# aerius-labs/indexed-merkle-tree-halo2

Hardware: AMD Instinct MI355X
Metric: indexed-tree insertions/sec at depth=32 (bn256::Fr) (higher is better)
Workload: dtype u32 limbs (9 x 29-bit, Montgomery mod p), 64-bit accumulate

## Files before the change

indexed-merkle-tree-halo2_amd/csrc/imt_device.hpp:

```cpp
#pragma once
#include <cstddef>
#include <cstdint>
#include "imt_consts.hpp"

#if defined(__HIPCC__)
#include <hip/hip_runtime.h>
#define IMT_HD __host__ __device__ __forceinline__
#else
#define IMT_HD inline
#endif

namespace imt {
namespace dev {

#define IMT_P29_0 0x10000001u
#define IMT_P29_1 0x1f0fac9fu
#define IMT_P29_2 0x0e5c2450u
#define IMT_P29_3 0x07d090f3u
#define IMT_P29_4 0x1585d283u
#define IMT_P29_5 0x02db40c0u
#define IMT_P29_6 0x00a6e141u
#define IMT_P29_7 0x0e5c2634u
#define IMT_P29_8 0x0030644eu
constexpr uint32_t N0INV29 = 0x0fffffffu;
constexpr uint32_t N0INV32 = 0xefffffffu;

IMT_HD constexpr uint32_t p29(int i) {
    return i == 0 ? IMT_P29_0 : i == 1 ? IMT_P29_1 : i == 2 ? IMT_P29_2 : i == 3 ? IMT_P29_3 :
           i == 4 ? IMT_P29_4 : i == 5 ? IMT_P29_5 : i == 6 ? IMT_P29_6 : i == 7 ? IMT_P29_7 : IMT_P29_8;
}


template <bool WIDE_M>
IMT_HD uint32_t mont_digit(uint64_t acc) {
    return WIDE_M ? (uint32_t)acc * N0INV32 : (((uint32_t)acc * N0INV29) & MASK29);
}

}
}
#if defined(__HIP_DEVICE_COMPILE__) && !defined(IMT_NO_MONT_ASM)
#define IMT_MONT_ASM 1
#include "imt_mont_asm.hpp"
#include "imt_mont_asm_rec.hpp"
#endif
namespace imt {
namespace dev {

template <int NT, bool ADD, bool WIDE_M = true>
IMT_HD void mont_dot(Fe& r, const Fe* a, const Fe* b, const Fe& addend) {
    uint32_t m[NL];
    uint64_t acc = 0;
#pragma unroll
    for (int k = 0; k < NL; k++) {
#pragma unroll
        for (int t = 0; t < NT; t++) {
#pragma unroll
            for (int i = 0; i <= k; i++) acc += (uint64_t)a[t].v[i] * b[t].v[k - i];
        }
#pragma unroll
        for (int i = 0; i < k; i++) acc += (uint64_t)m[i] * p29(k - i);
        m[k] = mont_digit<WIDE_M>(acc);
        acc += (uint64_t)m[k] * p29(0);
        acc >>= 29;
    }
#pragma unroll
    for (int k = NL; k < 2 * NL - 1; k++) {
#pragma unroll
        for (int t = 0; t < NT; t++) {
#pragma unroll
            for (int i = k - (NL - 1); i < NL; i++) acc += (uint64_t)a[t].v[i] * b[t].v[k - i];
        }
#pragma unroll
        for (int i = k - (NL - 1); i < NL; i++) acc += (uint64_t)m[i] * p29(k - i);
        if (ADD) acc += addend.v[k - NL];
        r.v[k - NL] = (uint32_t)acc & MASK29;
        acc >>= 29;
    }
    if (ADD) acc += addend.v[NL - 1];
    r.v[NL - 1] = (uint32_t)acc;
}

IMT_HD void mont_mul(Fe& r, const Fe& a, const Fe& b) {
#ifdef IMT_MONT_ASM
    masm::mul_vv(r, &a, &b);
#else
    mont_dot<1, false>(r, &a, &b, a);
#endif
}

template <int NT, bool ADD, bool WIDE_M = true>
IMT_HD void mont_dot_uc(Fe& r, const Fe* c, const Fe* v, const Fe& addend) {
#ifdef IMT_MONT_ASM
    static_assert((NT == 3 && !ADD && WIDE_M) || (NT == 4 && WIDE_M) || (NT == 2 && ADD && !WIDE_M),
                  "no assembly form for this shape");
    if constexpr (NT == 3) masm::dot3_uc(r, c, v);
    else if constexpr (NT == 4 && ADD) masm::dot4_add_uc(r, c, v, addend);
    else if constexpr (NT == 4) masm::dot4_uc(r, c, v);
    else masm::dot2_add_uc_narrow(r, c, v, addend);
#else
    mont_dot<NT, ADD, WIDE_M>(r, c, v, addend);
#endif
}

IMT_HD void mont_sqr(Fe& r, const Fe& a) {
#ifdef IMT_MONT_ASM
    masm::sqr_v(r, a);
    return;
#endif
    uint32_t m[NL], a2[NL];
#pragma unroll
    for (int i = 0; i < NL; i++) a2[i] = a.v[i] << 1;
    uint64_t acc = 0;
#pragma unroll
    for (int k = 0; k < NL; k++) {
#pragma unroll
        for (int i = 0; 2 * i < k; i++) acc += (uint64_t)a2[i] * a.v[k - i];
        if ((k & 1) == 0) acc += (uint64_t)a.v[k / 2] * a.v[k / 2];
#pragma unroll
        for (int i = 0; i < k; i++) acc += (uint64_t)m[i] * p29(k - i);
        m[k] = mont_digit<true>(acc);
        acc += (uint64_t)m[k] * p29(0);
        acc >>= 29;
    }
#pragma unroll
    for (int k = NL; k < 2 * NL - 1; k++) {
#pragma unroll
        for (int i = k - (NL - 1); 2 * i < k; i++) acc += (uint64_t)a2[i] * a.v[k - i];
        if ((k & 1) == 0) acc += (uint64_t)a.v[k / 2] * a.v[k / 2];
#pragma unroll
        for (int i = k - (NL - 1); i < NL; i++) acc += (uint64_t)m[i] * p29(k - i);
        r.v[k - NL] = (uint32_t)acc & MASK29;
        acc >>= 29;
    }
    r.v[NL - 1] = (uint32_t)acc;
}

IMT_HD void mont_redc(Fe& r, const Fe& a) {
    uint32_t m[NL];
    uint64_t acc = 0;
#pragma unroll
    for (int k = 0; k < NL; k++) {
        acc += a.v[k];
#pragma unroll
        for (int i = 0; i < k; i++) acc += (uint64_t)m[i] * p29(k - i);
        m[k] = mont_digit<false>(acc);
        acc += (uint64_t)m[k] * p29(0);
        acc >>= 29;
    }
#pragma unroll
    for (int k = NL; k < 2 * NL - 1; k++) {
#pragma unroll
        for (int i = k - (NL - 1); i < NL; i++) acc += (uint64_t)m[i] * p29(k - i);
        r.v[k - NL] = (uint32_t)acc & MASK29;
        acc >>= 29;
    }
    r.v[NL - 1] = (uint32_t)acc;
}

IMT_HD void add_lazy(Fe& r, const Fe& a, const Fe& b) {
#pragma unroll
    for (int i = 0; i < NL; i++) r.v[i] = a.v[i] + b.v[i];
}

IMT_HD void normalize(Fe& a) {
#pragma unroll
    for (int i = 0; i < NL - 1; i++) {
        a.v[i + 1] += a.v[i] >> 29;
        a.v[i] &= MASK29;
    }
}

IMT_HD bool geq_p(const Fe& a) {
    bool ge = true;
#pragma unroll
    for (int i = 0; i < NL; i++) {
        uint32_t pi = p29(i);
        if (a.v[i] != pi) ge = a.v[i] > pi;
    }
    return ge;
}

IMT_HD void sub_p(Fe& a) {
    uint32_t borrow = 0;
#pragma unroll
    for (int i = 0; i < NL; i++) {
        uint32_t d = a.v[i] - p29(i) - borrow;
        borrow = (i < NL - 1) ? (d >> 31) : 0;
        a.v[i] = (i < NL - 1) ? (d & MASK29) : d;
    }
}

template <int SH>
IMT_HD constexpr uint32_t p29_shl(int i) {
    return i == 0 ? ((p29(0) << SH) & MASK29)
         : i < NL - 1 ? (((p29(i) << SH) | (p29(i - 1) >> (29 - SH))) & MASK29)
                      : ((p29(i) << SH) | (p29(i - 1) >> (29 - SH)));
}
template <int SH>
IMT_HD void cond_sub_p_shl(Fe& a) {
    bool ge = true;
#pragma unroll
    for (int i = 0; i < NL; i++) {
        const uint32_t pi = p29_shl<SH>(i);
        if (a.v[i] != pi) ge = a.v[i] > pi;
    }
    if (ge) {
        uint32_t borrow = 0;
#pragma unroll
        for (int i = 0; i < NL; i++) {
            uint32_t d = a.v[i] - p29_shl<SH>(i) - borrow;
            borrow = (i < NL - 1) ? (d >> 31) : 0;
            a.v[i] = (i < NL - 1) ? (d & MASK29) : d;
        }
    }
}

IMT_HD void canonicalize(Fe& a) {
    cond_sub_p_shl<4>(a);
    cond_sub_p_shl<3>(a);
    cond_sub_p_shl<2>(a);
    cond_sub_p_shl<1>(a);
    cond_sub_p_shl<0>(a);
}

IMT_HD void unpack(Fe& r, const uint32_t w[8]) {
#pragma unroll
    for (int i = 0; i < NL; i++) {
        const int bit = 29 * i, wi = bit >> 5, sh = bit & 31;
        uint32_t lo = w[wi] >> sh;
        if (sh > 3 && wi + 1 < 8) lo |= w[wi + 1] << (32 - sh);
        r.v[i] = lo & MASK29;
    }
}
IMT_HD void pack(uint32_t w[8], const Fe& a) {
#pragma unroll
    for (int j = 0; j < 8; j++) {
        const int lo_limb = (32 * j) / 29, off = 32 * j - 29 * lo_limb;
        uint32_t x = a.v[lo_limb] >> off;
        const int have = 29 - off;
        if (have < 32 && lo_limb + 1 < NL) x |= a.v[lo_limb + 1] << have;
        if (have + 29 < 32 && lo_limb + 2 < NL) x |= a.v[lo_limb + 2] << (have + 29);
        w[j] = x;
    }
}

struct alignas(16) Word4 { uint32_t x, y, z, w; };
IMT_HD void load_packed(Fe& r, const void* ptr) {
    const Word4* q = reinterpret_cast<const Word4*>(ptr);
    Word4 x = q[0], y = q[1];
    uint32_t w[8] = {x.x, x.y, x.z, x.w, y.x, y.y, y.z, y.w};
    unpack(r, w);
}
IMT_HD void store_packed(void* ptr, const Fe& a) {
    uint32_t w[8];
    pack(w, a);
    Word4* q = reinterpret_cast<Word4*>(ptr);
    q[0] = Word4{w[0], w[1], w[2], w[3]};
    q[1] = Word4{w[4], w[5], w[6], w[7]};
}



IMT_HD void sbox(Fe& x) {
    Fe x2, x4;
    mont_sqr(x2, x);
    mont_sqr(x4, x2);
    mont_mul(x, x4, x);
}

IMT_HD constexpr uint32_t pc29(int i) { return i == 0 ? (1u << 29) - p29(0) : MASK29 - p29(i); }
constexpr uint32_t FOLD_RECIP = 1354;

IMT_HD void fold_p(Fe& a) {
    const uint32_t q = (uint32_t)(((uint64_t)a.v[NL - 1] * FOLD_RECIP) >> 32);
    uint64_t acc = 0;
#pragma unroll
    for (int i = 0; i < NL; i++) {
        acc = (acc >> 29) + a.v[i] + (uint64_t)q * pc29(i);
        a.v[i] = i < NL - 1 ? (uint32_t)acc & MASK29 : (uint32_t)(acc - ((uint64_t)q << 29));
    }
}

IMT_HD void permute(const PoseidonConsts& pc, Fe s[3], const Fe* first_rc) {
    constexpr int NSTEP = RF + RP;
    Fe z3;
#pragma unroll
    for (int i = 0; i < NL; i++) z3.v[i] = 0;
#pragma unroll 1
    for (int st = 0; st < NSTEP; st++) {
        if (st < RF / 2 || st >= RF / 2 + RP) {
            const int fr = st < RF / 2 ? st : st - RP;
            if (fr == RF / 2) {
                const Fe v[3] = {s[0], s[1], z3};
                const Fe zl = s[2];
#pragma unroll 1
                for (int i = 0; i < 2; i++) {
                    Fe n;
                    mont_dot_uc<3, false>(n, pc.rec_exit[i], v, v[0]);
                    add_lazy(n, n, zl);
                    normalize(n);
                    s[1] = s[2]; s[2] = n;
                }
            }
            const Fe* rc = (st == 0) ? first_rc : pc.sc_rc[fr];
            add_lazy(s[0], s[0], rc[0]);
            add_lazy(s[1], s[1], rc[1]);
            add_lazy(s[2], s[2], rc[2]);
            sbox(s[0]); sbox(s[1]); sbox(s[2]);
            const Fe(*mat)[3] = pc.sc_mats[fr];
            Fe n0, n1, n2;
            if (fr == 0 || fr == RF / 2) {
                mont_dot_uc<3, false>(n0, mat[0], s, s[0]);
            } else {
                add_lazy(n0, s[0], s[1]);
                add_lazy(n0, n0, s[2]);
                normalize(n0);
            }
            mont_dot_uc<3, false>(n1, mat[1], s, s[0]);
            mont_dot_uc<3, false>(n2, mat[2], s, s[0]);
            s[0] = n0; s[1] = n1; s[2] = n2;
        } else {
            const int r = st - RF / 2;
            Fe z, w;
            add_lazy(z, s[0], pc.rec_k[r]);
            sbox(z);
            if (r >= 2) {
                const Fe v[4] = {s[0], s[1], z3, s[2]};
                mont_dot_uc<4, true>(w, pc.rec_c[r], v, z);
            } else if (r == 1) {
                const Fe v[2] = {s[0], s[2]};
                Fe e;
                add_lazy(e, z3, z);
                mont_dot_uc<2, true, false>(w, pc.rec_c[1], v, e);
            } else {
                add_lazy(w, s[1], z);
                normalize(w);
            }
            s[1] = s[0]; s[0] = w; z3 = s[2]; s[2] = z;
        }
    }
}

IMT_HD void hash23(const PoseidonConsts& pc, Fe& out, const Fe& a, const Fe& b, const Fe& c, bool three) {
    Fe s[3] = {pc.cap0, a, b};
#pragma unroll 1
    for (int blk = 0; blk < 2; blk++) {
        const Fe* rc0 = pc.rc_full[0];
        if (blk == 1) {
            if (three) {
                add_lazy(s[1], s[1], c);
                add_lazy(s[2], s[2], pc.one);
                normalize(s[1]);
                normalize(s[2]);
            } else {
                rc0 = pc.rc_h2p2;
            }
        }
        permute(pc, s, rc0);
    }
    out = s[1];
    canonicalize(out);
}
IMT_HD void hash23_stashed(const PoseidonConsts& pc, Fe& out, const Fe& a, const Fe& b, bool three,
                           const uint32_t* stash, unsigned stride) {
    Fe s[3] = {pc.cap0, a, b};
#pragma unroll 1
    for (int blk = 0; blk < 2; blk++) {
        const Fe* rc0 = pc.rc_full[0];
        if (blk == 1) {
            if (three) {
                Fe c;
#pragma unroll
                for (int i = 0; i < NL; i++) c.v[i] = stash[(size_t)i * stride];
                add_lazy(s[1], s[1], c);
                add_lazy(s[2], s[2], pc.one);
                normalize(s[1]);
                normalize(s[2]);
            } else {
                rc0 = pc.rc_h2p2;
            }
        }
        permute(pc, s, rc0);
    }
    out = s[1];
    canonicalize(out);
}
IMT_HD void hash2(const PoseidonConsts& pc, Fe& out, const Fe& a, const Fe& b) { hash23(pc, out, a, b, a, false); }
IMT_HD void hash3(const PoseidonConsts& pc, Fe& out, const Fe& a, const Fe& b, const Fe& c) { hash23(pc, out, a, b, c, true); }

enum : unsigned { FMT_CANONICAL = 0, FMT_MONT256 = 1, FMT_DEVICE = 2 };

IMT_HD bool load_fe(const PoseidonConsts& pc, Fe& r, const void* ptr, unsigned fmt) {
    Fe raw;
    load_packed(raw, ptr);
    bool ok = !geq_p(raw) && (raw.v[NL - 1] >> 24) == 0;
    if (fmt == FMT_DEVICE) { r = raw; return ok; }
    mont_mul(r, raw, fmt == FMT_CANONICAL ? pc.from_canon : pc.from_mont256);
    canonicalize(r);
    return ok;
}
IMT_HD void store_fe(const PoseidonConsts& pc, void* ptr, const Fe& a, unsigned fmt) {
    if (fmt == FMT_DEVICE) { store_packed(ptr, a); return; }
    Fe t;
    mont_mul(t, a, fmt == FMT_CANONICAL ? pc.int_one : pc.to_mont256);
    canonicalize(t);
    store_packed(ptr, t);
}

IMT_HD bool fe_eq(const Fe& a, const Fe& b) {
    uint32_t d = 0;
#pragma unroll
    for (int i = 0; i < NL; i++) d |= a.v[i] ^ b.v[i];
    return d == 0;
}
IMT_HD bool fe_is_zero(const Fe& a) {
    uint32_t d = 0;
#pragma unroll
    for (int i = 0; i < NL; i++) d |= a.v[i];
    return d == 0;
}

}
}
```

indexed-merkle-tree-halo2_amd/csrc/imt_kernels.hip:

```cpp
#include <algorithm>
#include <hip/hip_runtime.h>
#include <hip/hip_ext.h>

#include "imt_device.hpp"
#include "imt_trace_device.hpp"
#include "imt_launch.hpp"
#include "imt_sweep.hpp"
#if defined(__HIP_DEVICE_COMPILE__)
#include "imt_coop_device.hpp"
#endif

namespace imt {

__constant__ dev::PoseidonConsts g_pc;
__constant__ dev::TraceConsts g_tc;

namespace {
using namespace dev;

#ifndef IMT_BLOCK
#define IMT_BLOCK 256
#endif
#ifndef IMT_HASH_WAVES
#define IMT_HASH_WAVES __attribute__((amdgpu_waves_per_eu(5, 5)))
// ... 417 lines not shown
        Fe rt;
        ok &= load_fe(g_pc, rt, root + i * (size_t)root_stride, fmt_in);
        if (!fe_eq(cur, rt)) fail |= 0x02;
        fail_out[i] = (uint8_t)fail;
        if (root_out) store_fe(g_pc, root_out + i * 32, cur, fmt_out);
    }
    flag_err(err, ok);
#endif
}

__global__ void __launch_bounds__(BLOCK) k_split128(const uint8_t* __restrict__ vals, uint8_t* __restrict__ q,
                                                    uint8_t* __restrict__ r, size_t n, unsigned fmt, int* err) {
    const size_t i = gtid();
    if (i >= n) return;
    Fe x, xi;
    bool ok = load_fe(g_pc, x, vals + i * 32, fmt);
    to_int(xi, x);
    uint32_t w[8];
    pack(w, xi);
    Fe lo, hi, t;
    const uint32_t wl[8] = {w[0], w[1], w[2], w[3], 0, 0, 0, 0};
    const uint32_t wh[8] = {w[4], w[5], w[6], w[7], 0, 0, 0, 0};
    unpack(t, wl);
    mont_mul(lo, t, g_pc.from_canon);
    canonicalize(lo);
    unpack(t, wh);
    mont_mul(hi, t, g_pc.from_canon);
    canonicalize(hi);
    store_fe(g_pc, r + i * 32, lo, fmt);
    store_fe(g_pc, q + i * 32, hi, fmt);
    flag_err(err, ok);
}

__global__ IMT_HASH_WAVES void __launch_bounds__(BLOCK)
k_insert_chains(const uint8_t* __restrict__ low_leaf, const uint64_t* __restrict__ low_index,
                const uint8_t* __restrict__ low_sib, const uint8_t* __restrict__ new_leaf,
                const uint64_t* __restrict__ new_index, const uint64_t* __restrict__ new_path_index,
                const uint8_t* __restrict__ new_sib, launch::SibLayout lay, unsigned depth, size_t n,
                uint8_t* __restrict__ trace, unsigned fmt_in, int* err) {
    const size_t i = gtid();
    if (i >= n) return;
    const int chain = blockIdx.y;
    __shared__ uint32_t stash[NL][BLOCK];
    bool ok = true;
    Fe cur;
    const uint8_t* sib = chain < 2 ? low_sib : new_sib;
    const uint64_t* index = chain < 2 ? low_index : new_path_index;
    const int leaf_row = chain == 0 ? 0 : chain == 1 ? 2 : 5, root_row = chain == 0 ? 1 : chain == 1 ? 3 : chain == 2 ? 4 : 6;
    if (chain == 2) cur = g_pc.zero_leaf;
    auto load_leaf = [=](Fe& a, Fe& b, Fe& c, bool& okk) {
        const size_t it = gtid_again();
        const uint8_t* const p0 = (chain == 3 ? new_leaf : low_leaf) + it * 96;
        okk &= load_fe(g_pc, a, p0, fmt_in);
        if (chain == 1) {
            okk &= load_fe(g_pc, b, new_leaf + it * 96, fmt_in);
            fe_from_u64(c, new_index[it]);
        } else {
            okk &= load_fe(g_pc, b, p0 + 32, fmt_in);
            okk &= load_fe(g_pc, c, p0 + 64, fmt_in);
        }
    };
    auto store_leaf = [=](const Fe& h) { store_packed(trace + ((size_t)leaf_row * n + gtid_again()) * 32, h); };
    chain_inline(cur, chain != 2, load_leaf, store_leaf, index, 0, sib, lay, depth, fmt_in, ok, &stash[0][threadIdx.x]);
    store_packed(trace + ((size_t)root_row * n + gtid_again()) * 32, cur);
    flag_err(err, ok);
}

__global__ IMT_COOP_WAVES void __launch_bounds__(BLOCK)
k_insert_chains_coop(const uint8_t* __restrict__ low_leaf, const uint64_t* __restrict__ low_index,
                     const uint8_t* __restrict__ low_sib, const uint8_t* __restrict__ new_leaf,
                     const uint64_t* __restrict__ new_index, const uint64_t* __restrict__ new_path_index,
                     const uint8_t* __restrict__ new_sib, launch::SibLayout lay, unsigned depth, size_t n,
                     uint8_t* __restrict__ trace, unsigned fmt_in, int* err) {
#if defined(__HIP_DEVICE_COMPILE__)
    __shared__ uint32_t tab[coop::TAB_DWORDS];
    coop::tab_fill(tab, g_pc);
    const size_t t = gtid();
    const size_t i = t >> 2;
    if (i >= n) return;
    const unsigned role = (unsigned)t & 3u, ri = role == 3u ? 0u : role;
    const int chain = blockIdx.y;
    bool ok = true;
    const uint8_t* sib = chain < 2 ? low_sib : new_sib;
    const uint64_t idx = chain < 2 ? low_index[i] : new_path_index[i];
    uint8_t* leaf_out = nullptr;
    uint8_t* root_out;
    Fe cur, X, C3, o;
    C3 = g_pc.one;
    if (chain == 2) {
        cur = g_pc.zero_leaf;
        root_out = trace + (4 * n + i) * 32;
    } else {
        if (chain == 1) {
            ok &= load_fe(g_pc, X, (ri == 2u ? new_leaf : low_leaf) + (i * 3 + 0) * 32, fmt_in);
            fe_from_u64(C3, new_index[i]);
            leaf_out = trace + (2 * n + i) * 32;
            root_out = trace + (3 * n + i) * 32;
        } else {
            const uint8_t* lf = chain == 0 ? low_leaf : new_leaf;
            ok &= load_fe(g_pc, X, lf + i * 96 + (ri == 2u ? 32 : 0), fmt_in);
            ok &= load_fe(g_pc, C3, lf + i * 96 + 64, fmt_in);
            if (ri == 1u) ok &= load_fe(g_pc, o, lf + i * 96 + 32, fmt_in);
            leaf_out = trace + ((chain == 0 ? 0 : 5) * n + i) * 32;
            root_out = trace + ((chain == 0 ? 1 : 6) * n + i) * 32;
        }
        coop::hash23(tab, o, X, C3, true, ri);
        coop::quad_bcast<1>(cur, o);
        if (role == 1u) store_packed(leaf_out, cur);
    }
#pragma unroll 1
    for (unsigned l = 0; l < depth; l++) {
        Fe sv;
        ok &= load_fe(g_pc, sv, sib + ((uint64_t)l * lay.level_stride + i * lay.item_stride) * 32, fmt_in);
        const bool right = (idx >> l) & 1;
        const bool take_sv = (ri == 2u) != right;
#pragma unroll
        for (int q = 0; q < NL; q++) X.v[q] = take_sv ? sv.v[q] : cur.v[q];
        coop::hash23(tab, o, X, C3, false, ri);
        coop::quad_bcast<1>(cur, o);
    }
    if (role == 1u) store_packed(root_out, cur);
    flag_err(err, ok);
#endif
}

__global__ void __launch_bounds__(BLOCK)
k_insert_check(const uint8_t* __restrict__ old_root, const uint8_t* __restrict__ low_leaf,
               const uint8_t* __restrict__ new_root, const uint8_t* __restrict__ new_leaf,
               const uint8_t* __restrict__ is_largest, size_t n, const uint8_t* __restrict__ trace,
               uint8_t* __restrict__ fail_out, unsigned fmt_in, int* err) {
    const size_t i = gtid();
    if (i >= n) return;
    bool ok = true;
    Fe low[3], nl[3], r0, r1, t;
#pragma unroll
    for (int j = 0; j < 3; j++) {
        ok &= load_fe(g_pc, low[j], low_leaf + (i * 3 + j) * 32, fmt_in);
        ok &= load_fe(g_pc, nl[j], new_leaf + (i * 3 + j) * 32, fmt_in);
    }
    ok &= load_fe(g_pc, r0, old_root + i * 32, fmt_in);
    ok &= load_fe(g_pc, r1, new_root + i * 32, fmt_in);
    unsigned fail = 0;
    Fe nvi, lvi, lni;
    to_int(nvi, nl[0]); to_int(lvi, low[0]); to_int(lni, low[1]);
    const unsigned s = is_largest[i];
    if (s > 1) fail |= 0x80;
    if (!(s ? fe_is_zero(low[1]) : int_lt(nvi, lni))) fail |= 0x01;
    if (!int_lt(lvi, nvi)) fail |= 0x04;
    load_packed(t, trace + (1 * n + i) * 32);
    if (!fe_eq(t, r0)) fail |= 0x02;
    Fe interim, z;
    load_packed(interim, trace + (3 * n + i) * 32);
    load_packed(z, trace + (4 * n + i) * 32);
    if (!fe_eq(z, interim)) fail |= 0x08;
    if (!fe_eq(nl[1], low[1])) fail |= 0x10;
    if (!fe_eq(nl[2], low[2])) fail |= 0x20;
    load_packed(t, trace + (6 * n + i) * 32);
    if (!fe_eq(t, r1)) fail |= 0x40;
    fail_out[i] = (uint8_t)fail;
    flag_err(err, ok);
}

__global__ IMT_HASH_WAVES void __launch_bounds__(BLOCK) k_tree_level(const uint8_t* __restrict__ prev, uint8_t* __restrict__ next,
                                                      size_t n_parents) {
    const size_t i = gtid();
    if (i >= n_parents) return;
    Fe a, b, o;
    load_packed(a, prev + (2 * i) * 32);
    load_packed(b, prev + (2 * i + 1) * 32);
    hash23_stashed(g_pc, o, a, b, false, nullptr, 0);
    store_packed(next + i * 32, o);
}

__device__ __forceinline__ void force_vector(Fe& x) {
#pragma unroll
    for (int i = 0; i < NL; i++) asm volatile("" : "+v"(x.v[i]));
}

__global__ IMT_HASH_WAVES void k_zero_chain(uint8_t* out, unsigned depth) {
#if defined(__HIP_DEVICE_COMPILE__)
    __shared__ uint32_t tab[coop::TAB_DWORDS];
    coop::tab_fill(tab, g_pc);
    if (blockIdx.x != 0 || threadIdx.x >= 4) return;
    const unsigned role = threadIdx.x, ri = role == 3u ? 0u : role;
    Fe cur = g_pc.zero_leaf;
    force_vector(cur);
    if (role == 1u) store_packed(out, cur);
#pragma unroll 1
    for (unsigned l = 0; l < depth; l++) {
        Fe o;
        coop::hash23(tab, o, cur, cur, false, ri);
        coop::quad_bcast<1>(cur, o);
        if (role == 1u) store_packed(out + (size_t)(l + 1) * 32, cur);
    }
#endif
}

__global__ IMT_HASH_WAVES void k_extend_root(uint8_t* cur_io, const uint8_t* zero, unsigned from, unsigned to) {
    if (threadIdx.x != 0 || blockIdx.x != 0) return;
    Fe cur;
    load_packed(cur, cur_io);
    force_vector(cur);
#pragma unroll 1
    for (unsigned l = from; l < to; l++) {
        Fe z, o;
        load_packed(z, zero + (size_t)l * 32);
        hash23_stashed(g_pc, o, cur, z, false, nullptr, 0);
        cur = o;
    }
    store_packed(cur_io, cur);
}

__global__ void __launch_bounds__(BLOCK) k_gather_proof(launch::TreeView tv, const uint64_t* __restrict__ index,
                                                        size_t n, unsigned depth, uint8_t* __restrict__ out,
                                                        launch::SibLayout lay, unsigned fmt_out) {
    const size_t t = gtid();
    if (t >= n * depth) return;
    const size_t i = t % n;
    const unsigned l = (unsigned)(t / n);
    const uint64_t s = ((index[i] - tv.index_base) >> l) ^ 1;
    const uint8_t* src = s < tv.len[l] ? tv.nodes + (tv.off[l] + s) * 32 : tv.zero + (size_t)l * 32;
    Fe x;
    load_packed(x, src);
    store_fe(g_pc, out + ((uint64_t)l * lay.level_stride + i * lay.item_stride) * 32, x, fmt_out);
}

__global__ void k_write_helpers(uint64_t index, unsigned depth, uint8_t* out, unsigned fmt_out) {
    const unsigned l = threadIdx.x + blockIdx.x * blockDim.x;
    if (l >= depth) return;
    Fe x;
    fe_from_u64(x, ((index >> l) & 1) ? 0 : 1);
    store_fe(g_pc, out + (size_t)l * 32, x, fmt_out);
}


__global__ void __launch_bounds__(BLOCK) k_fill_level(uint8_t* __restrict__ nodes, size_t n,
                                                      const uint8_t* __restrict__ zero_l) {
    const size_t i = gtid();
    if (i >= n) return;
    const Word4* z = reinterpret_cast<const Word4*>(zero_l);
    Word4* o = reinterpret_cast<Word4*>(nodes + i * 32);
    o[0] = z[0];
    o[1] = z[1];
}

__global__ void __launch_bounds__(BLOCK) k_merge_level(sweep::LevelTable in, sweep::LevelOut out, uint32_t total) {
    const size_t k = gtid();
    if (k >= total) return;
    sweep::merge_element(in, out, (uint32_t)k, total);
}

__global__ void __launch_bounds__(BLOCK)
k_writeback(const uint8_t* __restrict__ val_l, const uint32_t* __restrict__ from,
            const uint32_t* __restrict__ node_below, uint8_t* __restrict__ tree_l, uint32_t total) {
    const size_t kp = gtid();
    if (kp >= total) return;
    const uint32_t f = from[kp];
    if (!(f & sweep::LAST_BIT)) return;
    const Word4* s = reinterpret_cast<const Word4*>(val_l + (size_t)(f & ~sweep::LAST_BIT) * 32);
    Word4* d = reinterpret_cast<Word4*>(tree_l + (size_t)node_below[kp] * 32);
    d[0] = s[0];
    d[1] = s[1];
}

__global__ IMT_HASH_WAVES void __launch_bounds__(BLOCK) k_sweep(launch::SweepArgs a) {
    __shared__ uint32_t stash[NL][BLOCK];
    const size_t t = gtid();
    if (t >= a.count) return;
    const uint32_t x = a.begin + (uint32_t)t;
    Fe A, B, o;
    if (a.mode == launch::SWEEP_LEAVES) {
        const uint8_t* p = a.pre + (size_t)a.time0[x] * 96;
        Fe C;
        bool ok = load_fe(g_pc, A, p, a.fmt_in);
        ok &= load_fe(g_pc, B, p + 32, a.fmt_in);
        ok &= load_fe(g_pc, C, p + 64, a.fmt_in);
#pragma unroll
        for (int i = 0; i < NL; i++) stash[i][threadIdx.x] = C.v[i];
        flag_err(a.err, ok);
    } else {
        uint32_t k = x, n = 0, e = x;
        const uint8_t* sp = a.zero_l;
        if (a.from) {
            k = a.from[x] & ~sweep::LAST_BIT;
            n = a.node_below[x];
            e = a.time_next[x];
            const int32_t ss = a.sibsrc[x];
            const uint64_t sn = (uint64_t)(n ^ 1u);
            sp = ss >= 0 ? a.val_in + (size_t)ss * 32 : (sn < a.len_l ? a.tree_l + sn * 32 : a.zero_l);
        }
        Fe cur, sv;
        load_packed(cur, a.val_in + (size_t)k * 32);
        load_packed(sv, sp);
        if (x == a.last_event && a.node_in) store_packed(a.node_in, cur);
        const bool right = n & 1u;
#pragma unroll
        for (int i = 0; i < NL; i++) {
            A.v[i] = right ? sv.v[i] : cur.v[i];
            B.v[i] = right ? cur.v[i] : sv.v[i];
        }
        uint8_t* row = (e & 1u) ? a.new_sib : a.low_sib;
        if (row) store_fe(g_pc, row + ((uint64_t)a.level * a.lay.level_stride + (uint64_t)(e >> 1) * a.lay.item_stride) * 32, sv, a.fmt_out);
    }
    hash23_stashed(g_pc, o, A, B, a.mode == launch::SWEEP_LEAVES, &stash[0][threadIdx.x], BLOCK);
    store_packed(a.val_out + (size_t)x * 32, o);
    if (x == a.last_event && a.node_out) store_packed(a.node_out, o);
}

__global__ IMT_HASH_WAVES void __launch_bounds__(BLOCK) k_sweep_coop(launch::SweepArgs a) {
#if defined(__HIP_DEVICE_COMPILE__)
    __shared__ uint32_t tab[coop::TAB_DWORDS];
    coop::tab_fill(tab, g_pc);
    const size_t t = gtid();
    const size_t q = t >> 2;
    if (q >= a.count) return;
    const unsigned role = (unsigned)t & 3u, ri = role == 3u ? 0u : role;
    const uint32_t x = a.begin + (uint32_t)q;
    Fe X, C3, o;
    C3 = g_pc.one;
    if (a.mode == launch::SWEEP_LEAVES) {
        const uint8_t* p = a.pre + (size_t)a.time0[x] * 96;
        bool ok = load_fe(g_pc, X, p + (ri == 2u ? 32 : 0), a.fmt_in);
        ok &= load_fe(g_pc, C3, p + 64, a.fmt_in);
        if (ri == 1u) ok &= load_fe(g_pc, o, p + 32, a.fmt_in);
        flag_err(a.err, ok);
    } else {
        uint32_t k = x, n = 0, e = x;
        const uint8_t* sp = a.zero_l;
        if (a.from) {
            k = a.from[x] & ~sweep::LAST_BIT;
            n = a.node_below[x];
            e = a.time_next[x];
            const int32_t ss = a.sibsrc[x];
            const uint64_t sn = (uint64_t)(n ^ 1u);
            sp = ss >= 0 ? a.val_in + (size_t)ss * 32 : (sn < a.len_l ? a.tree_l + sn * 32 : a.zero_l);
        }
        Fe cur, sv;
        load_packed(cur, a.val_in + (size_t)k * 32);
        load_packed(sv, sp);
        const bool right = n & 1u;
        const bool take_sv = (ri == 2u) != right;
#pragma unroll
        for (int i = 0; i < NL; i++) X.v[i] = take_sv ? sv.v[i] : cur.v[i];
        if (role == 0u) {
            if (x == a.last_event && a.node_in) store_packed(a.node_in, cur);
            uint8_t* row = (e & 1u) ? a.new_sib : a.low_sib;
            if (row) store_fe(g_pc, row + ((uint64_t)a.level * a.lay.level_stride + (uint64_t)(e >> 1) * a.lay.item_stride) * 32, sv, a.fmt_out);
        }
    }
    coop::hash23(tab, o, X, C3, a.mode == launch::SWEEP_LEAVES, ri);
    if (role == 1u) {
        store_packed(a.val_out + (size_t)x * 32, o);
        if (x == a.last_event && a.node_out) store_packed(a.node_out, o);
    }
#endif
}

__global__ void __launch_bounds__(BLOCK)
k_emit_roots(const uint8_t* __restrict__ val, uint32_t e_begin, uint32_t e_count, uint32_t total,
             uint8_t* __restrict__ old_root, uint8_t* __restrict__ interim_root, uint8_t* __restrict__ new_root,
             unsigned fmt_out, uint8_t* __restrict__ roots_dev, uint8_t* __restrict__ node_store) {
    const size_t t = gtid();
    if (t >= e_count) return;
    const uint32_t e = e_begin + (uint32_t)t;
    Fe cur;
    load_packed(cur, val + (size_t)e * 32);
    if (e == total - 1 && node_store) store_packed(node_store, cur);
    if (roots_dev) { store_packed(roots_dev + (size_t)e * 32, cur); return; }
    const uint32_t i = e >> 1;
    if (e & 1u) {
        if (new_root) store_fe(g_pc, new_root + (size_t)i * 32, cur, fmt_out);
        if (old_root && (size_t)i + 1 < (size_t)(total >> 1)) store_fe(g_pc, old_root + ((size_t)i + 1) * 32, cur, fmt_out);
    } else {
        if (interim_root) store_fe(g_pc, interim_root + (size_t)i * 32, cur, fmt_out);
    }
}

__global__ IMT_HASH_WAVES void __launch_bounds__(BLOCK) k_apply_level(launch::ApplyArgs a) {
    __shared__ uint32_t stash[NL][BLOCK];
    const size_t j = gtid();
    if (j >= a.bound || j >= *a.count) return;
    const uint64_t p = a.list[j];
    if (p >= a.len_out) return;
    Fe A, B, o;
    if (a.mode == launch::APPLY_LEAVES) {
        const uint8_t* q = a.pre + (size_t)a.src[j] * 96;
        Fe C;
        bool ok = load_fe(g_pc, A, q, a.fmt_in);
        ok &= load_fe(g_pc, B, q + 32, a.fmt_in);
        ok &= load_fe(g_pc, C, q + 64, a.fmt_in);
#pragma unroll
        for (int i = 0; i < NL; i++) stash[i][threadIdx.x] = C.v[i];
        flag_err(a.err, ok);
    } else {
        const uint64_t c0 = 2 * p, c1 = 2 * p + 1;
        load_packed(A, c0 < a.len_in ? a.tree_in + c0 * 32 : a.zero_in);
        load_packed(B, c1 < a.len_in ? a.tree_in + c1 * 32 : a.zero_in);
    }
    hash23_stashed(g_pc, o, A, B, a.mode == launch::APPLY_LEAVES, &stash[0][threadIdx.x], BLOCK);
    store_packed(a.tree_out + p * 32, o);
}

__global__ IMT_HASH_WAVES void __launch_bounds__(BLOCK) k_apply_level_coop(launch::ApplyArgs a) {
#if defined(__HIP_DEVICE_COMPILE__)
    __shared__ uint32_t tab[coop::TAB_DWORDS];
    coop::tab_fill(tab, g_pc);
    const size_t t = gtid();
    const size_t j = t >> 2;
    if (j >= a.bound || j >= *a.count) return;
    const unsigned role = (unsigned)t & 3u, ri = role == 3u ? 0u : role;
    const uint64_t p = a.list[j];
    if (p >= a.len_out) return;
    Fe X, C3, o;
    C3 = g_pc.one;
    if (a.mode == launch::APPLY_LEAVES) {
        const uint8_t* q = a.pre + (size_t)a.src[j] * 96;
        bool ok = load_fe(g_pc, X, q + (ri == 2u ? 32 : 0), a.fmt_in);
        ok &= load_fe(g_pc, C3, q + 64, a.fmt_in);
        if (ri == 1u) ok &= load_fe(g_pc, o, q + 32, a.fmt_in);
        flag_err(a.err, ok);
    } else {
        const uint64_t ch = 2 * p + (ri == 2u ? 1u : 0u);
        load_packed(X, ch < a.len_in ? a.tree_in + ch * 32 : a.zero_in);
    }
    coop::hash23(tab, o, X, C3, a.mode == launch::APPLY_LEAVES, ri);
    if (role == 1u) store_packed(a.tree_out + p * 32, o);
#endif
}

__global__ IMT_HASH_WAVES void k_apply_top(uint8_t* nodes, const uint64_t* __restrict__ off, const uint64_t* __restrict__ len,
                                           const uint8_t* __restrict__ zero, unsigned from, unsigned to) {
#if defined(__HIP_DEVICE_COMPILE__)
    __shared__ uint32_t tab[coop::TAB_DWORDS];
    coop::tab_fill(tab, g_pc);
    if (blockIdx.x != 0 || threadIdx.x >= 4) return;
    const unsigned role = threadIdx.x, ri = role == 3u ? 0u : role;
    Fe cur;
    load_packed(cur, nodes + off[from] * 32);
#pragma unroll 1
    for (unsigned l = from; l < to; l++) {
        Fe z, X, o;
        load_packed(z, l == from && len[l] > 1 ? nodes + (off[l] + 1) * 32 : zero + (size_t)l * 32);
        coop::sel(X, ri == 2u, z, cur);
        coop::hash23(tab, o, X, X, false, ri);
        coop::quad_bcast<1>(cur, o);
        if (role == 1u) store_packed(nodes + off[l + 1] * 32, cur);
    }
#endif
}

__global__ IMT_HASH_WAVES void __launch_bounds__(BLOCK)
k_lift_roots(uint8_t* __restrict__ old_root, uint8_t* __restrict__ interim_root, uint8_t* __restrict__ new_root,
             uint32_t n, const uint8_t* __restrict__ top, uint64_t pos_bits, unsigned levels, unsigned fmt, int* err) {
    const size_t t = gtid();
    const uint32_t n_int = interim_root ? n : 0, n_new = new_root ? n : 0;
    const uint32_t n_old = old_root ? (new_root ? 1u : n) : 0;
    if (t >= (size_t)n_int + n_new + n_old) return;
    uint8_t* row;
    uint8_t* also = nullptr;
    if (t < n_int) {
        row = interim_root + t * 32;
    } else if (t < (size_t)n_int + n_new) {
        const size_t i = t - n_int;
        row = new_root + i * 32;
        if (old_root && i + 1 < n) also = old_root + (i + 1) * 32;
    } else {
        row = old_root + (t - n_int - n_new) * 32;
    }
    Fe cur;
    bool ok = load_fe(g_pc, cur, row, fmt);
#pragma unroll 1
    for (unsigned j = 0; j < levels; j++) {
        Fe sv, a, b, o;
        load_packed(sv, top + (size_t)j * 32);
        const bool right = (pos_bits >> j) & 1;
#pragma unroll
        for (int i = 0; i < NL; i++) {
            a.v[i] = right ? sv.v[i] : cur.v[i];
            b.v[i] = right ? cur.v[i] : sv.v[i];
        }
        hash23_stashed(g_pc, o, a, b, false, nullptr, 0);
        cur = o;
    }
    store_fe(g_pc, row, cur, fmt);
    if (also) store_fe(g_pc, also, cur, fmt);
    flag_err(err, ok);
}

__global__ void __launch_bounds__(BLOCK)
k_fill_sib_rows(uint8_t* __restrict__ sib, launch::SibLayout lay, unsigned first_level, unsigned levels, uint32_t n,
                const uint8_t* __restrict__ top, unsigned fmt_out) {
    const size_t t = gtid();
    if (t >= (size_t)n * levels) return;
    const uint32_t i = (uint32_t)(t % n);
    const unsigned j = (unsigned)(t / n);
    Fe x;
    load_packed(x, top + (size_t)j * 32);
    store_fe(g_pc, sib + ((uint64_t)(first_level + j) * lay.level_stride + (uint64_t)i * lay.item_stride) * 32, x, fmt_out);
}

__global__ void k_mix_roots(const uint8_t* __restrict__ before, const uint8_t* __restrict__ after,
                            uint8_t* __restrict__ mixed, uint32_t n_sub, uint32_t self, unsigned fmt_in, int* err) {
    const uint32_t r = blockIdx.x * blockDim.x + threadIdx.x;
    if (r >= n_sub) return;
    Fe x;
    const bool ok = load_fe(g_pc, x, (r < self ? after : before) + (size_t)r * 32, fmt_in);
    store_packed(mixed + (size_t)r * 32, x);
    flag_err(err, ok);
}

__global__ void k_pick_top(const uint8_t* __restrict__ levels_buf, uint32_t n_sub, uint32_t self, unsigned k,
                           unsigned levels, const uint8_t* __restrict__ zero, unsigned sub_depth,
                           uint8_t* __restrict__ top) {
    const unsigned j = threadIdx.x;
    if (j >= levels) return;
    const uint8_t* src;
    if (j < k) {
        const size_t off = 2 * (size_t)n_sub - ((2 * (size_t)n_sub) >> j);
        src = levels_buf + (off + ((self >> j) ^ 1u)) * 32;
    } else {
        src = zero + (size_t)(sub_depth + j) * 32;
    }
    const Word4* s4 = reinterpret_cast<const Word4*>(src);
    Word4* d4 = reinterpret_cast<Word4*>(top + (size_t)j * 32);
    d4[0] = s4[0];
    d4[1] = s4[1];
}

__global__ void __launch_bounds__(BLOCK) k_slot0(const uint32_t* __restrict__ time0, uint32_t* __restrict__ slot0,
                                                 uint32_t total) {
    const size_t k = gtid();
    if (k < total) slot0[time0[k]] = (uint32_t)k;
}

struct ExtractArgs {
    const uint8_t* const* val;
    const uint32_t* slot;
    const int32_t* sibsrc;
    const uint32_t* node_below;
    size_t stride;
    const uint8_t* tree_nodes;
    const uint64_t* tree_off;
    const uint64_t* tree_len;
    const uint8_t* zero;
    const uint8_t* roots;
    unsigned l0, depth;
    uint32_t ins_begin, ins_count, n_total;
    uint8_t *old_root, *interim_root, *new_root, *low_sib, *new_sib;
    launch::SibLayout lay;
    unsigned fmt_out;
};
__global__ void __launch_bounds__(BLOCK) k_extract(ExtractArgs a) {
    const size_t t = gtid();
    const size_t per = (size_t)a.depth + 1;
    if (t >= (size_t)a.ins_count * 2 * per) return;
    const uint32_t ev_local = (uint32_t)(t % ((size_t)a.ins_count * 2));
    const unsigned task = (unsigned)(t / ((size_t)a.ins_count * 2));
    const uint32_t i_local = ev_local >> 1, odd = ev_local & 1u;
    const uint32_t e = (a.ins_begin + i_local) * 2 + odd;
    Fe x;
    if (task == a.depth) {
        load_packed(x, a.roots + (size_t)e * 32);
        if (odd) {
            if (a.new_root) store_fe(g_pc, a.new_root + (size_t)i_local * 32, x, a.fmt_out);
        } else {
            if (a.interim_root) store_fe(g_pc, a.interim_root + (size_t)i_local * 32, x, a.fmt_out);
            if (a.old_root) {
                Fe o;
                if (e > 0) load_packed(o, a.roots + (size_t)(e - 1) * 32);
                else load_packed(o, a.tree_nodes + a.tree_off[a.depth] * 32);
                store_fe(g_pc, a.old_root + (size_t)i_local * 32, o, a.fmt_out);
            }
        }
        return;
    }
    uint8_t* dst = odd ? a.new_sib : a.low_sib;
    if (!dst) return;
    const unsigned l = task;
    const uint8_t* sp;
    if (l < a.l0) {
        const uint32_t kp = a.slot[(size_t)(l + 1) * a.stride + e];
        const int32_t ss = a.sibsrc[(size_t)l * a.stride + kp];
        const uint64_t sn = (uint64_t)(a.node_below[(size_t)l * a.stride + kp] ^ 1u);
        sp = ss >= 0 ? a.val[l] + (size_t)ss * 32
                     : (sn < a.tree_len[l] ? a.tree_nodes + (a.tree_off[l] + sn) * 32 : a.zero + (size_t)l * 32);
    } else {
        sp = a.zero + (size_t)l * 32;
    }
    load_packed(x, sp);
    store_fe(g_pc, dst + ((uint64_t)l * a.lay.level_stride + (uint64_t)i_local * a.lay.item_stride) * 32, x, a.fmt_out);
}

__global__ void __launch_bounds__(BLOCK)
k_pack_writeback(const uint8_t* __restrict__ val_l, const uint32_t* __restrict__ from, const uint32_t* __restrict__ node_below,
                 uint32_t total, uint8_t* __restrict__ tree_l, uint8_t* __restrict__ out_vals,
                 uint32_t* __restrict__ out_nodes, uint32_t* counter, uint32_t cap) {
    const size_t kp = gtid();
    const uint32_t f = kp < total ? from[kp] : 0u;
    const bool last = (f & sweep::LAST_BIT) != 0;
    const uint64_t mask = __ballot(last);
    if (!last) return;
    const unsigned lane = __lane_id();
    const int leader = __ffsll((unsigned long long)mask) - 1;
    uint32_t base = 0;
    if ((int)lane == leader) base = atomicAdd(counter, (uint32_t)__popcll(mask));
    base = __shfl(base, leader);
    const uint32_t i = base + (uint32_t)__popcll(mask & ((1ull << lane) - 1ull));
// ... 368 lines not shown
```

Baseline: 3.647 million.

## Unroll Poseidon partial rounds by three and fuse both permutation blocks in one loop

Restructures the Poseidon permutation used by the sweep hash kernel. Partial rounds run in a manually unrolled triple body, which removes per-round branching and register moves. The two absorb blocks run inside a single driver loop with a callback for the second absorption. This should cut loop and control overhead and let the compiler schedule across rounds, at the cost of larger code and possibly higher register pressure under the fixed waves-per-EU bound.

```diff
diff --git a/indexed-merkle-tree-halo2_amd/csrc/imt_device.hpp b/indexed-merkle-tree-halo2_amd/csrc/imt_device.hpp
--- a/indexed-merkle-tree-halo2_amd/csrc/imt_device.hpp
+++ b/indexed-merkle-tree-halo2_amd/csrc/imt_device.hpp
@@ -281,64 +281,127 @@
     }
 }
 
+enum PartialBody {
+    PARTIAL_SINGLE = 0,
+    PARTIAL_TRIPLE = 1
+};
+
+IMT_HD void permute_step(const PoseidonConsts& pc, Fe s[3], Fe& z3, int st, const Fe* first_rc) {
+    if (st < RF / 2 || st >= RF / 2 + RP) {
+        const int fr = st < RF / 2 ? st : st - RP;
+        if (fr == RF / 2) {
+            const Fe v[3] = {s[0], s[1], z3};
+            const Fe zl = s[2];
+#pragma unroll 1
+            for (int i = 0; i < 2; i++) {
+                Fe n;
+                mont_dot_uc<3, false>(n, pc.rec_exit[i], v, v[0]);
+                add_lazy(n, n, zl);
+                normalize(n);
+                s[1] = s[2]; s[2] = n;
+            }
+        }
+        const Fe* rc = (st == 0) ? first_rc : pc.sc_rc[fr];
+        add_lazy(s[0], s[0], rc[0]);
+        add_lazy(s[1], s[1], rc[1]);
+        add_lazy(s[2], s[2], rc[2]);
+        sbox(s[0]); sbox(s[1]); sbox(s[2]);
+        const Fe(*mat)[3] = pc.sc_mats[fr];
+        Fe n0, n1, n2;
+        if (fr == 0 || fr == RF / 2) {
+            mont_dot_uc<3, false>(n0, mat[0], s, s[0]);
+        } else {
+            add_lazy(n0, s[0], s[1]);
+            add_lazy(n0, n0, s[2]);
+            normalize(n0);
+        }
+        mont_dot_uc<3, false>(n1, mat[1], s, s[0]);
+        mont_dot_uc<3, false>(n2, mat[2], s, s[0]);
+        s[0] = n0; s[1] = n1; s[2] = n2;
+    } else {
+        const int r = st - RF / 2;
+        Fe z, w;
+        add_lazy(z, s[0], pc.rec_k[r]);
+        sbox(z);
+        if (r >= 2) {
+            const Fe v[4] = {s[0], s[1], z3, s[2]};
+            mont_dot_uc<4, true>(w, pc.rec_c[r], v, z);
+        } else if (r == 1) {
+            const Fe v[2] = {s[0], s[2]};
+            Fe e;
+            add_lazy(e, z3, z);
+            mont_dot_uc<2, true, false>(w, pc.rec_c[1], v, e);
+        } else {
+            add_lazy(w, s[1], z);
+            normalize(w);
+        }
+        s[1] = s[0]; s[0] = w; z3 = s[2]; s[2] = z;
+    }
+}
+
 IMT_HD void permute(const PoseidonConsts& pc, Fe s[3], const Fe* first_rc) {
     constexpr int NSTEP = RF + RP;
     Fe z3;
 #pragma unroll
     for (int i = 0; i < NL; i++) z3.v[i] = 0;
 #pragma unroll 1
-    for (int st = 0; st < NSTEP; st++) {
-        if (st < RF / 2 || st >= RF / 2 + RP) {
-            const int fr = st < RF / 2 ? st : st - RP;
-            if (fr == RF / 2) {
-                const Fe v[3] = {s[0], s[1], z3};
-                const Fe zl = s[2];
-#pragma unroll 1
-                for (int i = 0; i < 2; i++) {
-                    Fe n;
-                    mont_dot_uc<3, false>(n, pc.rec_exit[i], v, v[0]);
-                    add_lazy(n, n, zl);
-                    normalize(n);
-                    s[1] = s[2]; s[2] = n;
-                }
+    for (int st = 0; st < NSTEP; st++) permute_step(pc, s, z3, st, first_rc);
+}
+
+IMT_HD void partial_rounds3(const PoseidonConsts& pc, Fe s[3], Fe& z3, int r) {
+    Fe za, zb, zc, wa, wb, wc;
+    add_lazy(za, s[0], pc.rec_k[r]);
+    sbox(za);
+    {
+        const Fe v[4] = {s[0], s[1], z3, s[2]};
+        mont_dot_uc<4, true>(wa, pc.rec_c[r], v, za);
+    }
+    add_lazy(zb, wa, pc.rec_k[r + 1]);
+    sbox(zb);
+    {
+        const Fe v[4] = {wa, s[0], s[2], za};
+        mont_dot_uc<4, true>(wb, pc.rec_c[r + 1], v, zb);
+    }
+    add_lazy(zc, wb, pc.rec_k[r + 2]);
+    sbox(zc);
+    {
+        const Fe v[4] = {wb, wa, za, zb};
+        mont_dot_uc<4, true>(wc, pc.rec_c[r + 2], v, zc);
+    }
+    s[0] = wc; s[1] = wb; z3 = zb; s[2] = zc;
+}
+
+template <class Next>
+IMT_HD void permute_blocks3(const PoseidonConsts& pc, Fe s[3], const Fe* first_rc, Next next) {
+    constexpr int NSTEP = RF + RP, T0 = RF / 2 + 2, T1 = RF / 2 + RP - 1;
+    static_assert((T1 - T0) % 3 == 0, "the partial rounds after the seeds are triples plus round 56");
+    Fe z3;
+#pragma unroll
+    for (int i = 0; i < NL; i++) z3.v[i] = 0;
+    int st = 0;
+#pragma unroll 1
+    for (;;) {
+#pragma unroll 1
+        do {
+            if (st == NSTEP) {
+                if (!next(s, first_rc)) return;
+                st = 0;
             }
-            const Fe* rc = (st == 0) ? first_rc : pc.sc_rc[fr];
-            add_lazy(s[0], s[0], rc[0]);
-            add_lazy(s[1], s[1], rc[1]);
-            add_lazy(s[2], s[2], rc[2]);
-            sbox(s[0]); sbox(s[1]); sbox(s[2]);
-            const Fe(*mat)[3] = pc.sc_mats[fr];
-            Fe n0, n1, n2;
-            if (fr == 0 || fr == RF / 2) {
-                mont_dot_uc<3, false>(n0, mat[0], s, s[0]);
-            } else {
-                add_lazy(n0, s[0], s[1]);
-                add_lazy(n0, n0, s[2]);
-                normalize(n0);
-            }
-            mont_dot_uc<3, false>(n1, mat[1], s, s[0]);
-            mont_dot_uc<3, false>(n2, mat[2], s, s[0]);
-            s[0] = n0; s[1] = n1; s[2] = n2;
-        } else {
-            const int r = st - RF / 2;
-            Fe z, w;
-            add_lazy(z, s[0], pc.rec_k[r]);
-            sbox(z);
-            if (r >= 2) {
-                const Fe v[4] = {s[0], s[1], z3, s[2]};
-                mont_dot_uc<4, true>(w, pc.rec_c[r], v, z);
-            } else if (r == 1) {
-                const Fe v[2] = {s[0], s[2]};
-                Fe e;
-                add_lazy(e, z3, z);
-                mont_dot_uc<2, true, false>(w, pc.rec_c[1], v, e);
-            } else {
-                add_lazy(w, s[1], z);
-                normalize(w);
-            }
-            s[1] = s[0]; s[0] = w; z3 = s[2]; s[2] = z;
-        }
-    }
+            permute_step(pc, s, z3, st, first_rc);
+            st++;
+        } while (st != T0);
+#pragma unroll 1
+        do {
+            partial_rounds3(pc, s, z3, st - RF / 2);
+            st += 3;
+        } while (st != T1);
+    }
+}
+
+template <PartialBody PB>
+IMT_HD void permute(const PoseidonConsts& pc, Fe s[3], const Fe* first_rc) {
+    if constexpr (PB == PARTIAL_TRIPLE) permute_blocks3(pc, s, first_rc, [](Fe*, const Fe*&) { return false; });
+    else permute(pc, s, first_rc);
 }
 
 IMT_HD void hash23(const PoseidonConsts& pc, Fe& out, const Fe& a, const Fe& b, const Fe& c, bool three) {
@@ -361,9 +424,36 @@
     out = s[1];
     canonicalize(out);
 }
+IMT_HD void absorb_stashed(const PoseidonConsts& pc, Fe s[3], const Fe*& rc0, bool three, const uint32_t* stash,
+                           unsigned stride) {
+    if (three) {
+        Fe c;
+#pragma unroll
+        for (int i = 0; i < NL; i++) c.v[i] = stash[(size_t)i * stride];
+        add_lazy(s[1], s[1], c);
+        add_lazy(s[2], s[2], pc.one);
+        normalize(s[1]);
+        normalize(s[2]);
+    } else {
+        rc0 = pc.rc_h2p2;
+    }
+}
+template <PartialBody PB = PARTIAL_SINGLE>
 IMT_HD void hash23_stashed(const PoseidonConsts& pc, Fe& out, const Fe& a, const Fe& b, bool three,
                            const uint32_t* stash, unsigned stride) {
     Fe s[3] = {pc.cap0, a, b};
+    if constexpr (PB == PARTIAL_TRIPLE) {
+        bool second = true;
+        permute_blocks3(pc, s, pc.rc_full[0], [&](Fe* t, const Fe*& rc0) {
+            if (!second) return false;
+            second = false;
+            absorb_stashed(pc, t, rc0, three, stash, stride);
+            return true;
+        });
+        out = s[1];
+        canonicalize(out);
+        return;
+    }
 #pragma unroll 1
     for (int blk = 0; blk < 2; blk++) {
         const Fe* rc0 = pc.rc_full[0];
diff --git a/indexed-merkle-tree-halo2_amd/csrc/imt_kernels.hip b/indexed-merkle-tree-halo2_amd/csrc/imt_kernels.hip
--- a/indexed-merkle-tree-halo2_amd/csrc/imt_kernels.hip
+++ b/indexed-merkle-tree-halo2_amd/csrc/imt_kernels.hip
@@ -743,7 +743,7 @@
         uint8_t* row = (e & 1u) ? a.new_sib : a.low_sib;
         if (row) store_fe(g_pc, row + ((uint64_t)a.level * a.lay.level_stride + (uint64_t)(e >> 1) * a.lay.item_stride) * 32, sv, a.fmt_out);
     }
-    hash23_stashed(g_pc, o, A, B, a.mode == launch::SWEEP_LEAVES, &stash[0][threadIdx.x], BLOCK);
+    hash23_stashed<PARTIAL_TRIPLE>(g_pc, o, A, B, a.mode == launch::SWEEP_LEAVES, &stash[0][threadIdx.x], BLOCK);
     store_packed(a.val_out + (size_t)x * 32, o);
     if (x == a.last_event && a.node_out) store_packed(a.node_out, o);
 }
```

New measurement: 3.664 million (median of 6 runs). Within noise of the previous version (+0.4%).
